# YangHai-1218/SCFlow

Measured on AMD Instinct MI355X. Metric: image-pairs/sec at 256x256, 8 GRU iters, higher is better.
Workload: dtype f32

## Files before the change

include/scflow_hip_prof.h:

```cpp
#ifndef SCFLOW_HIP_PROF_H
#define SCFLOW_HIP_PROF_H

#include "scflow_hip.h"

#ifdef __cplusplus
extern "C" {
#endif

typedef void* scf_timer_t;
int scf_timer_create(scf_timer_t* timer);
int scf_timer_destroy(scf_timer_t timer);
int scf_timer_elapsed_us(scf_timer_t timer, float* microseconds);
int scf_timer_arm(scf_timer_t timer);

int scf_conv2d_query(const scf_conv_desc* desc, int32_t* info);

enum {
  SCF_KERNEL_THIN = 1,
  SCF_KERNEL_TAPS = 2,
  SCF_KERNEL_WINO = 3,
  SCF_KERNEL_WINO1D = 4,
  SCF_KERNEL_F16X3 = 5,
  SCF_KERNEL_DMA = 6,
  SCF_KERNEL_MFMA = 7,
  SCF_KERNEL_MFMA_KSPLIT = 8,
  SCF_KERNEL_WINO_Q = 9,
  SCF_KERNEL_WINO1D4 = 10
};
typedef struct scf_conv_log_entry {
  int32_t kernel;
  int32_t Cin, Cout, KH, KW, stride, Ho, Wo, N;
  int32_t mode;
  int32_t paired;
  int32_t variant;
} scf_conv_log_entry;
int scf_conv_log_enable(int capacity);
enum {
  SCF_TUNE_WINO_VARIANT = 1,
  SCF_TUNE_DMA_FORCE_KSPLIT = 2,
  SCF_TUNE_DMA_KSPLIT_GROUPS = 3,
  SCF_TUNE_WINO1D4 = 4,
  SCF_TUNE_CONV_AUTOSLICE = 7,
  SCF_TUNE_LOOKUP_STORE = 6,
  SCF_TUNE_ITER_MERGE = 8,
  SCF_TUNE_WINO1D4_HALF = 9,
  SCF_TUNE_CONV_PAIR = 10,
  SCF_TUNE_LOOKUP_PIPE = 5
};
int scf_tune(int key, int value);
int scf_conv_log_read(scf_conv_log_entry* out, int max_entries);

#ifdef __cplusplus
}
#endif
#endif
```

scflow_amd/csrc/conv_mfma.hip:

```cpp
#include <atomic>
#include <mutex>
#include <vector>
#include "scf_common.h"

typedef float f32x16 __attribute__((ext_vector_type(16)));
typedef float f32x4 __attribute__((ext_vector_type(4)));

#include "conv_kernels.h"

template <int WM, int WN, int NCP>
__device__ __forceinline__ void mfma_taps(f32x16 (&acc)[WM][WN], const float* wl, const float* pl,
                                          const int (&boff)[WN], int T, int KW, int KC, int BM,
                                          int PW, int PHW, int half, int l32) {
  for (int t = 0; t < T; ++t) {
    const int ky = t / KW, kx = t - ky * KW;
    const float* wt = wl + (t * KC + half) * BM + l32;
    const float* pt = pl + ky * PW + kx;
#pragma unroll
    for (int c = 0; c < NCP; ++c) {
      const int cp = 2 * c;
      float a[WM], b[WN];
#pragma unroll
      for (int i = 0; i < WM; ++i) a[i] = wt[cp * BM + i * 32];
#pragma unroll
// ... 503 lines not shown

static int conv2d_walk(const scf_conv_desc* d, scf_stream_t stream, ConvReq& r) {
  ConvPlan pl;
  const int rc = conv_plan(d, &pl);
  if (rc != SCF_OK) return rc;
  const ConvK& k = pl.k;
  const int N = d->N;
  const bool dry = r.info || r.cap;
  int32_t scratch[4];
  int32_t* info = r.info ? r.info : r.cap ? scratch : nullptr;
  hipStream_t st = scf_stream(stream);
  int out = SCF_EUNSUPPORTED;
  auto took = [&](int which, int rf) { r.which = which; out = rf; return rf != SCF_EUNSUPPORTED; };
  if (d->k_slices > 1) {
    r.which = SCF_KERNEL_DMA;
    return want_dma(d) ? scf_conv_dma_dispatch(k, N, dry, info, st, r.cap) : SCF_EUNSUPPORTED;
  }
  if (took(SCF_KERNEL_THIN, scf_conv_thin_dispatch(k, N, dry, st, r.cap))) return out;
  if (d->wp_taps && took(SCF_KERNEL_TAPS, scf_conv_taps_dispatch(k, d->wp_taps, N, dry, info, st, r.cap))) return out;
  if (d->wp_wino) {
    int quarter = 0;
    const int rw = scf_conv_wino_dispatch(k, d->wp_wino, N, dry, info, st, &quarter, r.cap);
    if (took(quarter ? SCF_KERNEL_WINO_Q : SCF_KERNEL_WINO, rw)) return out;
  }
  const int w4 = g_wino1d4.load(std::memory_order_relaxed);
  if (d->wp_wino1d4 && w4 && took(SCF_KERNEL_WINO1D4, scf_conv_wino1d4_dispatch(k, d->wp_wino1d4, N, w4 == 2, dry, info, st)))
    return out;
  if (d->wp_wino1d && took(SCF_KERNEL_WINO1D, scf_conv_wino1d_dispatch(k, d->wp_wino1d, N, dry, info, st))) return out;
  if (want_f16x3(d) && took(SCF_KERNEL_F16X3, scf_conv_f16x3_dispatch(k, N, dry, info, st))) return out;
  if (want_dma(d)) {
    float* ws = nullptr;
    int64_t ws_floats = 0;
    const bool sliced = !r.info && g_autoslice.load(std::memory_order_relaxed) && kws_lookup(st, &ws, &ws_floats);
    if (sliced && !dry) {
      const int S = scf_conv_dma_autoslice(k, N);
      const int64_t per_slice = (int64_t)N * d->Cout * k.Ho * k.Wo;
      if (S > 1 && per_slice * S <= ws_floats) {
        ConvK part = k;
        part.out = ws; part.out_ns = (long long)d->Cout * k.Ho * k.Wo;
        part.bias = nullptr; part.scale = nullptr; part.shift = nullptr; part.res = nullptr; part.res_ns = 0;
        part.out_div = 1.f; part.out_div_pow2 = 1; part.act = SCF_ACT_NONE; part.act2 = SCF_ACT_NONE; part.act_split = 0;
        part.mode = SCF_CONV_PLAIN; part.gru_h = nullptr; part.gru_aux = nullptr; part.gru_z = nullptr;
        part.kslices = S; part.slice_ns = per_slice;
        r.which = SCF_KERNEL_DMA;
        const int rs = scf_conv_dma_dispatch(part, N, false, nullptr, st);
        if (rs == SCF_OK) return scf_conv_kcombine_launch(k, ws, S, per_slice, N, st);
        if (rs != SCF_EUNSUPPORTED) return rs;
      }
    }
    if (took(SCF_KERNEL_DMA, scf_conv_dma_dispatch(k, N, dry, info, st, r.cap))) {
      if (sliced && r.cap) r.cap->variant = -1;
      return out;
    }
  }
  r.which = k.ksplit ? SCF_KERNEL_MFMA_KSPLIT : SCF_KERNEL_MFMA;
  const int WM = pl.WM, WN = pl.WN;
  if (dry) {
    if (r.info) {
      r.info[0] = WM; r.info[1] = WN; r.info[2] = (int32_t)pl.nblk;
      r.info[3] = k.T * (k.KC / 2) * WM * WN / (k.ksplit ? 4 : 1);
    }
    return SCF_OK;
  }
  const int nblk = (int)pl.nblk;
  if (k.ksplit) {
    if (k.KC == 32) return launch_ksplit<32>(k, nblk, pl.lds_bytes, st);
    if (k.KC == 8) return launch_ksplit<8>(k, nblk, pl.lds_bytes, st);
    return launch_ksplit<2>(k, nblk, pl.lds_bytes, st);
  }
#define SCF_CASE(M, Nn) if (WM == M && WN == Nn) return launch_conv<M, Nn>(k, nblk, pl.lds_bytes, st);
  SCF_CASE(1, 1) SCF_CASE(1, 2) SCF_CASE(2, 1) SCF_CASE(2, 2)
  SCF_CASE(3, 1) SCF_CASE(4, 1)
#undef SCF_CASE
  return SCF_EUNSUPPORTED;
}

namespace {
std::mutex g_log_mu;
std::vector<scf_conv_log_entry> g_log;
std::atomic<int> g_log_cap{0};
}

int scf_wino_variant_set(int v);
int scf_dma_force_ksplit_set(int v);
int scf_dma_ksplit_groups_set(int v);
int scf_lookup_pipe_set(int v);
int scf_lookup_store_set(int v);
int scf_iter_merge_set(int v);
int scf_wino1d4_half_set(int v);

extern "C" int scf_tune(int key, int value) {
  if (key == SCF_TUNE_WINO_VARIANT) return scf_wino_variant_set(value);
  if (key == SCF_TUNE_DMA_FORCE_KSPLIT) return scf_dma_force_ksplit_set(value);
  if (key == SCF_TUNE_DMA_KSPLIT_GROUPS) return scf_dma_ksplit_groups_set(value);
  if (key == SCF_TUNE_LOOKUP_PIPE) return scf_lookup_pipe_set(value);
  if (key == SCF_TUNE_LOOKUP_STORE) return scf_lookup_store_set(value);
  if (key == SCF_TUNE_ITER_MERGE) return scf_iter_merge_set(value);
  if (key == SCF_TUNE_WINO1D4_HALF) return scf_wino1d4_half_set(value);
  if (key == SCF_TUNE_CONV_AUTOSLICE) {
    if (value < 0 || value > 1) return SCF_EINVAL;
    return g_autoslice.exchange(value);
  }
  if (key == SCF_TUNE_CONV_PAIR) {
    if (value < 0 || value > 1) return SCF_EINVAL;
    return g_pair_mode.exchange(value);
  }
  if (key == SCF_TUNE_WINO1D4) {
    if (value < 0 || value > 2) return SCF_EINVAL;
    return g_wino1d4.exchange(value);
  }
  return SCF_EINVAL;
}

extern "C" int scf_conv_log_enable(int capacity) {
  std::lock_guard<std::mutex> lk(g_log_mu);
  g_log.clear();
  if (capacity > 0) g_log.reserve((size_t)capacity);
  else g_log.shrink_to_fit();
  g_log_cap.store(capacity > 0 ? capacity : 0);
  return SCF_OK;
}

extern "C" int scf_conv_log_read(scf_conv_log_entry* out, int max_entries) {
  std::lock_guard<std::mutex> lk(g_log_mu);
  const int n = (int)g_log.size();
  if (out)
    for (int i = 0; i < n && i < max_entries; ++i) out[i] = g_log[(size_t)i];
  return n;
}

static void conv_log_push(const scf_conv_desc* d, int which, int paired, int variant = -1);
extern "C" int scf_conv2d(const scf_conv_desc* d, scf_stream_t stream) {
  ConvReq r;
  const int rc = conv2d_walk(d, stream, r);
  if (rc == SCF_OK) conv_log_push(d, r.which, 0);
  return rc;
}

static void conv_log_push(const scf_conv_desc* d, int which, int paired, int variant) {
  if (g_log_cap.load(std::memory_order_relaxed) <= 0) return;
  std::lock_guard<std::mutex> lk(g_log_mu);
  if ((int)g_log.size() >= g_log_cap.load()) return;
  scf_conv_log_entry e;
  e.kernel = which; e.Cin = d->C0 + d->C1; e.Cout = d->Cout; e.KH = d->KH; e.KW = d->KW; e.stride = d->stride;
  e.Ho = (d->H + 2 * d->pad_h - d->KH) / d->stride + 1;
  e.Wo = (d->W + 2 * d->pad_w - d->KW) / d->stride + 1;
  e.N = d->N; e.mode = d->mode; e.paired = paired; e.variant = variant;
  g_log.push_back(e);
}

static bool pairable(int which, const ScfLaunchCap& c) {
  switch (which) {
    case SCF_KERNEL_THIN: return true;
    case SCF_KERNEL_TAPS: return c.variant >= 1;
    case SCF_KERNEL_WINO_Q: return c.variant >= 10 && c.variant < 20;
    case SCF_KERNEL_WINO: return c.variant >= 20;
    case SCF_KERNEL_DMA: return c.variant >= 0;
    default: return false;
  }
}

static bool capture(const scf_conv_desc* d, scf_stream_t stream, ScfLaunchCap* cap, int* which) {
  ConvReq r;
  r.cap = cap;
  const bool ok = conv2d_walk(d, stream, r) == SCF_OK && pairable(r.which, *cap);
  *which = r.which;
  return ok;
}

typedef int (*PairLaunch)(const ScfLaunchCap&, const ScfLaunchCap&, hipStream_t);

static bool shared_input_form(const scf_conv_desc* a, const scf_conv_desc* b) {
  return a->in0 == b->in0 && a->C1 == 0 && b->C1 == 0 && a->C0 == b->C0 && a->N == b->N && a->H == b->H && a->W == b->W &&
         a->in0_nstride == b->in0_nstride && a->KH == 3 && a->KW == 3 && a->stride == 2 && a->pad_h == 1 && a->pad_w == 1 &&
         b->KH == 1 && b->KW == 1 && b->stride == 2 && b->pad_h == 0 && b->pad_w == 0;
// ... 158 lines not shown
```

scflow_amd/csrc/conv_wino.hip:

```cpp
#include <stdlib.h>
#include <string.h>
#include "scf_common.h"
#include "conv_kernels.h"
#include "scf_dma.h"

typedef float wn_f32x16 __attribute__((ext_vector_type(16)));
typedef float wn_f32x4 __attribute__((ext_vector_type(4)));
typedef float wn_f32x2 __attribute__((ext_vector_type(2)));

#define WN_NPI(TW, PX4) ((PX4) ? ((TW) == 2 ? 3 : 2) : ((TW) == 2 ? 8 : 5))
#define WN_KC 4
#ifndef SCF_WINO_DEFAULT_VARIANT
#define SCF_WINO_DEFAULT_VARIANT 2
#endif

#ifdef SCF_WINO_LAB
#include "wino_lab_hooks.h"
#else
#define WN_LAB(bit) 0
#define WN_LAB_FIELDS
#endif

struct WinoK {
  const float* wu;
// ... 513 lines not shown

  float* box = wn_lds + tw * (4 * 3072);
  const int cb = (f0 + (row >> 1)) * 32 + 16 * (row & 1) + 4 * half;
  float bv[8], sc[8], sh[8];
#pragma unroll
  for (int k = 0; k < 8; ++k) {
    const int co = cb + 8 * (k >> 2) + (k & 3);
    const int cc = co < p.Cout ? co : 0;
    bv[k] = p.bias ? p.bias[cc] : 0.f;
    sc[k] = p.scale ? p.scale[cc] : 1.f;
    sh[k] = p.scale ? p.shift[cc] : 0.f;
  }
  __builtin_amdgcn_sched_barrier(0);
  wn_f32x4 own[4];
#pragma unroll
  for (int qq = 0; qq < 32; qq += 2) {
    wn_f32x4 t;
#pragma unroll
    for (int h2 = 0; h2 < 2; ++h2) {
      const int f = (qq + h2) >> 4, r = (qq + h2) & 15;
      const float m0 = acc[4 * f][r], m1 = acc[4 * f + 1][r], m2 = acc[4 * f + 2][r], m3 = acc[4 * f + 3][r];
      t[2 * h2] = (m0 + m1) + m2;
      t[2 * h2 + 1] = (m1 - m2) - m3;
    }
    const int d = qq >> 3, kp = (qq & 7) >> 1;
    if (d == row) own[kp] = t;
    else *reinterpret_cast<wn_f32x4*>(box + (((row * 3 + (d < row ? d : d - 1)) * 4 + kp) * 64 + lane) * 4) = t;
  }
  __syncthreads();

  const ConvEpi e = scf_conv_epi(p, n);
  const int oy = y0 + 2 * ty, ox = x0 + 2 * tx;
  if (ox >= p.Wo || oy >= p.Ho || WN_LAB(3)) return;
  const bool row1 = oy + 1 < p.Ho;
  const bool relu = p.act == SCF_ACT_RELU;
  wn_f32x4 in[4][4];
#pragma unroll
  for (int sw = 0; sw < 4; ++sw)
#pragma unroll
    for (int kp = 0; kp < 4; ++kp) {
      if (sw == row) in[sw][kp] = own[kp];
      else in[sw][kp] = *reinterpret_cast<const wn_f32x4*>(box + (((sw * 3 + (row < sw ? row : row - 1)) * 4 + kp) * 64 + lane) * 4);
    }
  wn_f32x2 rr[8][2];
#pragma unroll
  for (int k = 0; k < 8; ++k) {
    const int co = cb + 8 * (k >> 2) + (k & 3);
    const int cc = co < p.Cout ? co : 0;
    const int off = cc * e.HWo + oy * p.Wo + ox;
#pragma unroll
    for (int i = 0; i < 2; ++i)
      rr[k][i] = (e.res && (i == 0 || row1)) ? *reinterpret_cast<const wn_f32x2*>(e.res + off + i * p.Wo) : wn_f32x2{0.f, 0.f};
  }
  __builtin_amdgcn_sched_barrier(0);
#pragma unroll
  for (int k = 0; k < 8; ++k) {
    const int co = cb + 8 * (k >> 2) + (k & 3);
    if (co >= p.Cout) continue;
    const int kp = k >> 1, h2 = 2 * (k & 1);
    wn_f32x2 y[2];
#pragma unroll
    for (int cI = 0; cI < 2; ++cI) {
      const float t0 = in[0][kp][h2 + cI], t1 = in[1][kp][h2 + cI], t3 = in[2][kp][h2 + cI], t2 = in[3][kp][h2 + cI];
      y[0][cI] = (t0 + t1) + t2;
      y[1][cI] = (t1 - t2) - t3;
    }
    const int off = co * e.HWo + oy * p.Wo + ox;
#pragma unroll
    for (int i = 0; i < 2; ++i) {
      if (i == 1 && !row1) break;
      wn_f32x2 v = {y[i][0] + bv[k], y[i][1] + bv[k]};
      if (p.scale) { v[0] = v[0] * sc[k] + sh[k]; v[1] = v[1] * sc[k] + sh[k]; }
      v[0] += rr[k][i][0]; v[1] += rr[k][i][1];
      if (relu) { v[0] = v[0] > 0.f ? v[0] : 0.f; v[1] = v[1] > 0.f ? v[1] : 0.f; }
      scf_store2<(SCF_ST_SC1 & 8) != 0>(e.out + off + i * p.Wo, v[0], v[1]);
    }
  }
}

template <int TW, bool PX4, int NR = 3, bool BURST = false>
__global__ __launch_bounds__(256 * TW, TW == 1 ? 2 : 1)
void conv_wino_q_kernel(ConvK p, WinoK q) {
  conv_wino_q_body<TW, PX4, NR, BURST>(p, q, (int)blockIdx.x, (int)gridDim.x);
}

template <bool PX4>
__global__ __launch_bounds__(256, 2)
void conv_wino_q_pair_kernel(ConvK pa, WinoK qa, ConvK pb, WinoK qb, int nba) {
  if ((int)blockIdx.x < nba) conv_wino_q_body<1, PX4>(pa, qa, (int)blockIdx.x, nba);
  else conv_wino_q_body<1, PX4>(pb, qb, (int)blockIdx.x - nba, (int)gridDim.x - nba);
}

template <bool PXA, bool PXB>
__global__ __launch_bounds__(256, 2)
void conv_wino_mixed_pair_kernel(ConvK pa, WinoK qa, ConvK pb, WinoK qb, int nba) {
  if ((int)blockIdx.x < nba) conv_wino_q_body<1, PXA>(pa, qa, (int)blockIdx.x, nba);
  else conv_wino_body<1, 2, PXB>(pb, qb, (int)blockIdx.x - nba, (int)gridDim.x - nba);
}

extern "C" int64_t scf_pack_conv_weight_wino_size(int32_t cout, int32_t cin) {
  if (cout <= 0 || cin <= 0) return 0;
  const int64_t F = (cout + 31) / 32, nchunk = (cin + WN_KC - 1) / WN_KC;
  return nchunk * 16 * F * 128;
}

extern "C" int scf_pack_conv_weight_wino(const float* w, int32_t cout, int32_t cin, float* out) {
  if (!w || !out || cout <= 0 || cin <= 0) return SCF_EINVAL;
  const int F = (cout + 31) / 32;
  memset(out, 0, sizeof(float) * (size_t)scf_pack_conv_weight_wino_size(cout, cin));
  static const double G[4][3] = {{1.0, 0.0, 0.0}, {0.5, 0.5, 0.5}, {0.5, -0.5, 0.5}, {0.0, 0.0, 1.0}};
  for (int co = 0; co < cout; ++co)
    for (int ci = 0; ci < cin; ++ci) {
      const float* g = w + ((size_t)co * cin + ci) * 9;
      double t[4][3];
      for (int i = 0; i < 4; ++i)
        for (int b = 0; b < 3; ++b) t[i][b] = G[i][0] * g[b] + G[i][1] * g[3 + b] + G[i][2] * g[6 + b];
      const int chunk = ci / WN_KC, cl = ci % WN_KC, s = cl >> 1, kh = cl & 1;
      const int frag = co / 32, m = co % 32;
      for (int i = 0; i < 4; ++i)
        for (int j = 0; j < 4; ++j) {
          const double u = t[i][0] * G[j][0] + t[i][1] * G[j][1] + t[i][2] * G[j][2];
          const int pos = 4 * (i < 2 ? i : 5 - i) + j;
          out[(((size_t)chunk * F + frag) * 16 + pos) * 128 + kh * 64 + m * 2 + s] = (float)u;
        }
    }
  return SCF_OK;
}

static std::atomic<int> g_wino_variant{0};
int scf_wino_variant_set(int v) {
#ifndef SCF_WINO_LAB
  if (v < 0 || v > 2) return SCF_EINVAL;
#else
  if (v < 0 || v > 5) return SCF_EINVAL;
#endif
  return g_wino_variant.exchange(v);
}

int scf_conv_wino_dispatch(ConvK k, const float* wu, int N, bool dry_run, int* info, hipStream_t st, int* which, ScfLaunchCap* cap) {
  if (which) *which = 0;
  if (!wu || k.KH != 3 || k.KW != 3 || k.stride != 1 || k.pad_h != 1 || k.pad_w != 1) return SCF_EUNSUPPORTED;
  if (k.w_ns != 0 || k.out_tile || k.mode != SCF_CONV_PLAIN || k.out_div != 1.0f || k.act_split > 0) return SCF_EUNSUPPORTED;
  if (k.act != SCF_ACT_NONE && k.act != SCF_ACT_RELU) return SCF_EUNSUPPORTED;
  if ((k.Wo & 1) || (k.out_ns & 1) || ((uintptr_t)k.out & 7) || (k.res && ((k.res_ns & 1) || ((uintptr_t)k.res & 7)))) return SCF_EUNSUPPORTED;
  if (k.in1 && (k.C0 % WN_KC) != 0) return SCF_EUNSUPPORTED;
  if (((uintptr_t)wu & 15) || (long long)WN_KC * k.H * k.W * 4 >= 0x7fffffffLL) return SCF_EUNSUPPORTED;
  const int F = (k.Cout + 31) / 32;
  const int tcols = (k.Wo + 1) / 2;
  int txl = 4;
  {
    int best = (tcols + 15) / 16 * 16;
    if (tcols < 16) { txl = 0; while ((1 << txl) < tcols) ++txl; if (txl < 2) txl = 2; best = 0; }
    for (int l = 3; l >= 2 && best; --l) {
      const int wpad = (tcols + (1 << l) - 1) >> l << l;
      if (wpad * 10 <= best * 9) { best = wpad; txl = l; }
    }
  }
  const int TXW = 1 << txl, TYW = 32 >> txl;
  const bool px4 = (k.W % 4) == 0 && (((uintptr_t)k.in0 | (uintptr_t)k.in1) & 15) == 0 && (k.in0_ns % 4) == 0 && (k.in1_ns % 4) == 0;
  const int cfg = px4 ? 1 : 0;
  WinoK q;
  q.wu = wu; q.F = F; q.txl = txl;
  q.nchunk = (k.Cin + WN_KC - 1) / WN_KC;
  q.sx = (k.Wo + 2 * TXW - 1) / (2 * TXW);
  auto shape = [&](int CW, int TW, int pslot) -> long long {
    q.PH = 2 * TW * TYW + 2; q.PW = px4 ? 2 * TXW + 8 : 2 * TXW + 2;
    q.PWp = q.PW + ((TXW - q.PW) & 31);
    if (WN_KC * q.PH * q.PWp > pslot) q.PWp = q.PW;
    q.PPL = q.PH * q.PWp;
    if (WN_KC * q.PPL > pslot || (F % CW) != 0) return -1;
    q.sy = (k.Ho + 2 * TW * TYW - 1) / (2 * TW * TYW);
    q.mblocks = F / CW;
    const long long nblk = (long long)N * q.sx * q.sy * q.mblocks;
    return (nblk <= 0 || nblk > 0x7fffffffLL) ? -1 : nblk;
  };
  const int min_blocks4 = scf_cu_count() / 2;
  int variant = g_wino_variant.load(std::memory_order_relaxed);
  if (variant == 0) variant = SCF_WINO_DEFAULT_VARIANT;
#ifndef SCF_WINO_LAB
  if (variant >= 3) variant = 2;
#endif
  if (variant == 2 || variant == 3 || variant == 4 || variant == 5) {
    const int TW = variant == 3 ? 2 : 1;
    const int NR = variant >= 4 ? 4 : 3;
    const bool burst = variant == 5; (void)burst;
    const int npi = WQ_NPI(TW, px4), pslot = npi * 256 * TW * (px4 ? 4 : 1);
    const long long nblk = shape(2, TW, pslot);
    if (nblk > 0 && nblk * TW >= min_blocks4) {
      if (which) *which = 1;
      size_t ldsf = (size_t)NR * (2 * 2048 + pslot);
      if (ldsf < (size_t)TW * 4 * 3072) ldsf = (size_t)TW * 4 * 3072;
      const size_t ldsb = ldsf * sizeof(float);
      if (info) { info[0] = 16; info[1] = 2 * TW; info[2] = (int)nblk; info[3] = (int)ldsb; }
      if (cap) {
        static_assert(sizeof(WinoK) <= sizeof(cap->aux), "ScfLaunchCap::aux holds a WinoK");
        cap->k = k; cap->nblk = (int)nblk; cap->ldsb = ldsb;
        memcpy(cap->aux, &q, sizeof(WinoK));
        cap->variant = (TW == 1 && NR == 3) ? 10 + cfg : -1;
        return SCF_OK;
      }
      if (dry_run) return SCF_OK;
      static std::atomic<unsigned long long> raised_q[4];
#ifdef SCF_WINO_LAB
      if (TW == 2) {
        const void* fn8 = cfg ? (const void*)conv_wino_q_kernel<2, true> : (const void*)conv_wino_q_kernel<2, false>;
        const int rc8 = scf_raise_dynamic_lds(raised_q[2 + cfg], fn8, 96 * 1024);
        if (rc8 != SCF_OK) return rc8;
        if (cfg) scf_launch((conv_wino_q_kernel<2, true>), dim3((unsigned)nblk), dim3(512), ldsb, st, k, q);
        else scf_launch((conv_wino_q_kernel<2, false>), dim3((unsigned)nblk), dim3(512), ldsb, st, k, q);
        return scf_launch_status();
      }
#endif
#ifdef SCF_WINO_LAB
      if (NR == 4 && burst) {
        static std::atomic<unsigned long long> raised_qb[2];
        const void* fnb = cfg ? (const void*)conv_wino_q_kernel<1, true, 4, true> : (const void*)conv_wino_q_kernel<1, false, 4, true>;
        const int rcb = scf_raise_dynamic_lds(raised_qb[cfg], fnb, 80 * 1024);
        if (rcb != SCF_OK) return rcb;
        if (cfg) scf_launch((conv_wino_q_kernel<1, true, 4, true>), dim3((unsigned)nblk), dim3(256), ldsb, st, k, q);
        else scf_launch((conv_wino_q_kernel<1, false, 4, true>), dim3((unsigned)nblk), dim3(256), ldsb, st, k, q);
        return scf_launch_status();
      }
      if (NR == 4) {
        static std::atomic<unsigned long long> raised_q4[2];
        const void* fn4 = cfg ? (const void*)conv_wino_q_kernel<1, true, 4> : (const void*)conv_wino_q_kernel<1, false, 4>;
        const int rc4 = scf_raise_dynamic_lds(raised_q4[cfg], fn4, 80 * 1024);
        if (rc4 != SCF_OK) return rc4;
        if (cfg) scf_launch((conv_wino_q_kernel<1, true, 4>), dim3((unsigned)nblk), dim3(256), ldsb, st, k, q);
        else scf_launch((conv_wino_q_kernel<1, false, 4>), dim3((unsigned)nblk), dim3(256), ldsb, st, k, q);
        return scf_launch_status();
      }
#endif
      const void* fn = cfg ? (const void*)conv_wino_q_kernel<1, true> : (const void*)conv_wino_q_kernel<1, false>;
      const int rc = scf_raise_dynamic_lds(raised_q[cfg], fn, 64 * 1024);
      if (rc != SCF_OK) return rc;
      if (cfg) scf_launch((conv_wino_q_kernel<1, true>), dim3((unsigned)nblk), dim3(256), ldsb, st, k, q);
      else scf_launch((conv_wino_q_kernel<1, false>), dim3((unsigned)nblk), dim3(256), ldsb, st, k, q);
      return scf_launch_status();
    }
  }
  const int CW = 1, TW = 2;
  const int npi = WN_NPI(TW, px4);
  const long long nblk = shape(CW, TW, npi * (px4 ? 1024 : 256));
  if (nblk < 0) return SCF_EUNSUPPORTED;
  if (nblk < min_blocks4) return SCF_EUNSUPPORTED;
  const size_t ldsb = (size_t)(3 * CW * 2048 + 3 * npi * (px4 ? 1024 : 256)) * sizeof(float);
  if (ldsb > 80 * 1024) return SCF_EUNSUPPORTED;
  if (info) { info[0] = 16; info[1] = CW * TW; info[2] = (int)nblk; info[3] = (int)ldsb; }
  if (cap) {
    cap->k = k; cap->nblk = (int)nblk; cap->ldsb = ldsb;
    memcpy(cap->aux, &q, sizeof(WinoK));
    cap->variant = 20 + cfg;
    return SCF_OK;
  }
  if (dry_run) return SCF_OK;
  {
    static std::atomic<unsigned long long> raised[2];
    const int rc = scf_raise_dynamic_lds(raised[cfg], cfg ? (const void*)conv_wino_kernel<1, 2, true>
                                                          : (const void*)conv_wino_kernel<1, 2, false>, 80 * 1024);
    if (rc != SCF_OK) return rc;
  }
  if (cfg) scf_launch((conv_wino_kernel<1, 2, true>), dim3((unsigned)nblk), dim3(256), ldsb, st, k, q);
  else scf_launch((conv_wino_kernel<1, 2, false>), dim3((unsigned)nblk), dim3(256), ldsb, st, k, q);
  return scf_launch_status();
}

int scf_conv_wino_pair_launch(const ScfLaunchCap& a, const ScfLaunchCap& b, hipStream_t st) {
  if (a.variant >= 10 && a.variant < 20 && b.variant >= 20 && a.nblk > 0 && b.nblk > 0) {
    const size_t ldsm = a.ldsb > b.ldsb ? a.ldsb : b.ldsb;
    WinoK qa, qb;
    memcpy(&qa, a.aux, sizeof(WinoK));
    memcpy(&qb, b.aux, sizeof(WinoK));
    const int ca = a.variant - 10, cb2 = b.variant - 20, id = ca * 2 + cb2;
    static std::atomic<unsigned long long> raised_m[4];
    const void* fn = id == 0 ? (const void*)conv_wino_mixed_pair_kernel<false, false> : id == 1 ? (const void*)conv_wino_mixed_pair_kernel<false, true>
                   : id == 2 ? (const void*)conv_wino_mixed_pair_kernel<true, false> : (const void*)conv_wino_mixed_pair_kernel<true, true>;
    const int rc = scf_raise_dynamic_lds(raised_m[id], fn, 80 * 1024);
    if (rc != SCF_OK) return rc;
    const dim3 grid((unsigned)(a.nblk + b.nblk));
    if (id == 0) scf_launch((conv_wino_mixed_pair_kernel<false, false>), grid, dim3(256), ldsm, st, a.k, qa, b.k, qb, a.nblk);
    else if (id == 1) scf_launch((conv_wino_mixed_pair_kernel<false, true>), grid, dim3(256), ldsm, st, a.k, qa, b.k, qb, a.nblk);
    else if (id == 2) scf_launch((conv_wino_mixed_pair_kernel<true, false>), grid, dim3(256), ldsm, st, a.k, qa, b.k, qb, a.nblk);
    else scf_launch((conv_wino_mixed_pair_kernel<true, true>), grid, dim3(256), ldsm, st, a.k, qa, b.k, qb, a.nblk);
    return scf_launch_status();
  }
  if (a.variant < 10 || a.variant >= 20 || a.variant != b.variant || a.nblk <= 0 || b.nblk <= 0) return SCF_EUNSUPPORTED;
  const size_t lds = a.ldsb > b.ldsb ? a.ldsb : b.ldsb;
  WinoK qa, qb;
  memcpy(&qa, a.aux, sizeof(WinoK));
  memcpy(&qb, b.aux, sizeof(WinoK));
  const int cfg = a.variant - 10;
  static std::atomic<unsigned long long> raised[2];
  const void* fn = cfg ? (const void*)conv_wino_q_pair_kernel<true> : (const void*)conv_wino_q_pair_kernel<false>;
  const int rc = scf_raise_dynamic_lds(raised[cfg], fn, 64 * 1024);
  if (rc != SCF_OK) return rc;
  const unsigned grid = (unsigned)(a.nblk + b.nblk);
  if (cfg) scf_launch((conv_wino_q_pair_kernel<true>), dim3(grid), dim3(256), lds, st, a.k, qa, b.k, qb, a.nblk);
  else scf_launch((conv_wino_q_pair_kernel<false>), dim3(grid), dim3(256), lds, st, a.k, qa, b.k, qb, a.nblk);
  return scf_launch_status();
}
```

scflow_amd/ops.py:

```python
from __future__ import annotations

import ctypes as C
import os
import math
from dataclasses import dataclass
from typing import List, Optional, Sequence, Tuple

import torch

from . import _lib
from ._lib import (ACT_NONE, ACT_RELU, ACT_SIGMOID, ACT_TANH, CONV_GRU_Q, CONV_GRU_ZR,
                   CONV_PLAIN, ConvDesc)

Tensor = torch.Tensor

__all__ = ['record_conv_kernels', 'PackedConv', 'conv_desc', 'gru_passes', 'scflow_iteration', 'side_stream_handle', 'pyramid_layout', 'untile_level', 'level_storage_shape', 'sepconv_gru', 'pack_conv_weight', 'pack_conv_weight_f16x3', 'set_conv_precision', 'set_conv_winograd', 'get_conv_winograd', 'pack_conv_weight_wino', 'pack_conv_weight_wino1d', 'pack_conv_weight_wino1d4',
           'get_conv_precision', 'set_conv_kslices', 'conv_kslices', 'conv_kslices_for', 'constant', 'clear_constants', 'register_conv_workspace', 'choose_kc', 'conv2d', 'conv2d_pair', 'corr_build', 'corr_lookup',
           'instance_norm', 'group_norm_relu', 'linear', 'fc_splitk', 'fc_slices', 'pose_update', 'reproject_flow',
           'flow_corr_2d3d', 'pnp_params', 'pnp_ransac', 'pnp',
           'unproject_depth', 'linear_pair', 'resize_bilinear', 'resize_bilinear_grad', 'reproject_flow_grad', 'pose_update_grad', 'convex_upsample', 'avgpool2x2', 'copy_channels',
           'fc_operand', 'fc_dgrad', 'fc_wgrad', 'pose_select_grad', 'group_norm_flat_grad',
           'ACT_NONE', 'ACT_RELU', 'ACT_SIGMOID', 'ACT_TANH', 'CONV_PLAIN', 'CONV_GRU_ZR',
           'CONV_GRU_Q']

# ... 579 lines not shown
            g.wp_zr_a4s, g.wp_q_a4s, g.a4s_groups = pzr.wp4s.data_ptr(), pq.wp4s.data_ptr(), pzr.g4s
        if pzr.wp4t is not None and pq.wp4t is not None and pzr.g4t == pq.g4t:
            g.wp_zr_a4t, g.wp_q_a4t, g.a4t_groups = pzr.wp4t.data_ptr(), pq.wp4t.data_ptr(), pzr.g4t
        if _CONV_WINOGRAD and not f16 and pzr.wwino1d is not None and pq.wwino1d is not None:
            g.wp_zr_wino1d, g.wp_q_wino1d = pzr.wwino1d.data_ptr(), pq.wwino1d.data_ptr()
            if pzr.wwino1d4 is not None and pq.wwino1d4 is not None:
                g.wp_zr_wino1d4, g.wp_q_wino1d4 = pzr.wwino1d4.data_ptr(), pq.wwino1d4.data_ptr()
    return arr


gru_passes = _gru_passes


def side_stream_handle() -> int:
    main = torch.cuda.current_stream()
    key = (torch.cuda.current_device(), main.cuda_stream)
    side = _SIDE.get(key)
    if side is None:
        side = _SIDE[key] = torch.cuda.Stream(device=key[0])
    return side.cuda_stream


def scflow_iteration(it: '_lib.ScflowIter') -> None:
    lib = _lib.load()
    it.lookup_timer = _LOOKUP_TIMERS.take() if _LOOKUP_TIMERS is not None else None
    _lib.check(lib.scf_scflow_iteration(C.byref(it), _stream()), 'scf_scflow_iteration')


def sepconv_gru(packs, hx: Tensor, h_channels: int, z: Tensor, rh: Tensor,
                ctx: Optional[Sequence[Tensor]] = None, ctx_channels: int = 0) -> None:
    hc = h_channels
    if ctx is not None and (ctx_channels <= 0 or len(ctx) != len(packs)):
        raise _lib.ScflowHipError('sepconv_gru: one context term per pass, ctx_channels > 0')
    if _CONV_EVENTS is not None:
        hv, xv = hx[:, :hc], hx[:, hc + ctx_channels:]
        for i, (pzr, pq) in enumerate(packs):
            if ctx is None:
                conv2d(pzr, hx, out=z, mode=CONV_GRU_ZR, gru_h=hv, gru_aux=rh)
                conv2d(pq, rh, xv, out=hv, mode=CONV_GRU_Q, gru_h=hv, gru_z=z)
            else:
                conv2d(pzr, hv, xv, out=z, mode=CONV_GRU_ZR, gru_h=hv, gru_aux=rh, res=ctx[i][:, :2 * hc])
                conv2d(pq, rh, xv, out=hv, mode=CONV_GRU_Q, gru_h=hv, gru_z=z, res=ctx[i][:, 2 * hc:])
        return
    p, n, c, h, w, sn = _nchw(hx, 'hx')
    arr = _gru_passes(packs)
    if ctx is None:
        _lib.check(_lib.load().scf_sepconv_gru(p, sn, n, hc, c - hc, h, w, arr, len(packs),
                                               _dense(z, 'z'), _dense(rh, 'rh'), _stream()),
                   'scf_sepconv_gru')
        return
    ptrs, cs = (C.c_void_p * len(ctx))(), None
    for i, t in enumerate(ctx):
        pc_, nc, cc_, hh, ww, s_ = _nchw(t, 'ctx')
        if (nc, cc_, hh, ww) != (n, 3 * hc, h, w) or (cs is not None and s_ != cs):
            raise _lib.ScflowHipError('sepconv_gru: ctx must be (N, 3*h_channels, H, W), equal strides')
        ptrs[i], cs = pc_, s_
    _lib.check(_lib.load().scf_sepconv_gru_ctx(p, sn, n, hc, ctx_channels, c - hc - ctx_channels, h, w,
                                               arr, len(packs), ptrs, cs, _dense(z, 'z'),
                                               _dense(rh, 'rh'), _stream()),
               'scf_sepconv_gru_ctx')


def _read_timers(timers):
    lib = _lib.load()
    out = []
    for tm in timers:
        us = C.c_float()
        _lib.check(lib.scf_timer_elapsed_us(tm, C.byref(us)), 'scf_timer_elapsed_us')
        lib.scf_timer_destroy(tm)
        out.append(float(us.value))
    return out


def conv_timing(enable: bool):
    global _CONV_EVENTS
    if enable:
        _CONV_EVENTS = []
        return None
    evs, _CONV_EVENTS = _CONV_EVENTS or [], None
    torch.cuda.synchronize()
    return list(zip(_read_timers([e[0] for e in evs]), [e[1] for e in evs], [e[2] for e in evs]))


TUNE_KEYS = {'wino_variant': 1, 'dma_force_ksplit': 2, 'dma_ksplit_groups': 3, 'wino1d4': 4, 'lookup_pipe': 5, 'lookup_store': 6, 'conv_autoslice': 7, 'iter_merge': 8, 'wino1d4_half': 9, 'conv_pair': 10}


def tune(key: str, value: int) -> int:
    if key not in TUNE_KEYS:
        raise ValueError(f'unknown tune key {key!r}; known: {sorted(TUNE_KEYS)}')
    prev = int(_lib.load().scf_tune(TUNE_KEYS[key], int(value)))
    if prev < 0:
        _lib.check(prev, f'scf_tune({key}, {value})')
    return prev


class record_conv_kernels:

    _active = False

    def __init__(self, capacity: int = 1 << 16) -> None:
        self.capacity, self.ran, self.paired, self.variants = capacity, [], [], []

    def __enter__(self):
        if record_conv_kernels._active:
            raise RuntimeError('record_conv_kernels does not nest (one process-wide dispatch log)')
        _lib.check(_lib.load().scf_conv_log_enable(self.capacity), 'scf_conv_log_enable')
        record_conv_kernels._active = True
        return self.ran

    def __exit__(self, *exc):
        record_conv_kernels._active = False
        lib = _lib.load()
        n = lib.scf_conv_log_read(None, 0)
        buf = (_lib.ConvLogEntry * max(n, 1))()
        n = min(lib.scf_conv_log_read(buf, n), n)
        lib.scf_conv_log_enable(0)
        for e in buf[:n]:
            self.ran.append((f'{e.Cin}->{e.Cout} {e.KH}x{e.KW}/s{e.stride} @{e.Ho}x{e.Wo} N{e.N}',
                             _lib.KERNEL_NAMES.get(e.kernel, str(e.kernel))))
            self.paired.append(e.paired)
            self.variants.append(e.variant)
        return False


def time_first_kernel(fn) -> float:
    lib = _lib.load()
    tm = C.c_void_p()
    _lib.check(lib.scf_timer_create(C.byref(tm)), 'scf_timer_create')
    lib.scf_timer_arm(tm)
    try:
        fn()
    finally:
        lib.scf_timer_arm(None)
    torch.cuda.synchronize()
    return _read_timers([tm])[0]


def pyramid_layout(h: int, w: int, radius: int = 4, num_levels: int = 4) -> int:
    return int(_lib.load().scf_corr_preferred_layout(h, w, radius, num_levels))


def level_storage_shape(h: int, w: int, level: int, tiled: bool) -> Tuple[int, int]:
    lh, lw = h >> level, w >> level
    return ((lh + 3) // 4 * 4, (lw + 7) // 8 * 8) if tiled else (lh, lw)


def untile_level(level: Tensor, lh: int, lw: int) -> Tensor:
    q, _, ph, pw = level.shape
    return (level.reshape(q, ph // 4, pw // 8, 4, 8).permute(0, 1, 3, 2, 4).reshape(q, 1, ph, pw)
            [:, :, :lh, :lw].contiguous())


def untile_level0(level0: Tensor) -> Tensor:
    return untile_level(level0, level0.shape[-2], level0.shape[-1])


def _pyramid_shapes(n: int, h: int, w: int, num_levels: int, tiled_levels: int):
    return [(n * h * w, 1, *level_storage_shape(h, w, l, bool((tiled_levels >> l) & 1)))
            for l in range(num_levels)]


def corr_build(feat1: Tensor, feat2: Tensor, num_levels: int = 4,
               out: Optional[List[Tensor]] = None, tiled_levels: int = 0) -> List[Tensor]:
    p1 = _dense(feat1, 'feat1')
    p2 = _dense(feat2, 'feat2')
    if feat1.shape != feat2.shape or feat1.dim() != 4:
        raise _lib.ScflowHipError('feat1/feat2 must be equal-shape NCHW')
# ... 1238 lines not shown
```

Before: 2352.

## Add persistent tile-looping Winograd conv kernel overlapping next-tile loads with epilogue

Adds a persistent variant of the quantized Winograd conv kernel. It launches two blocks per CU and loops over tiles. During the tail chunks of the current tile it prefetches the next tile's patch and weight data into the LDS rings, and it reuses the U ring as the exchange box, so loads overlap the epilogue and stores. Stores use buffer_store with out-of-bounds masking. It is enabled by default when there are more blocks than slots. This adds scheduling complexity and risks exposing the serial epilogue, with fewer blocks to hide latency.

```diff
diff --git a/include/scflow_hip_prof.h b/include/scflow_hip_prof.h
--- a/include/scflow_hip_prof.h
+++ b/include/scflow_hip_prof.h
@@ -45,6 +45,7 @@
   SCF_TUNE_ITER_MERGE = 8,
   SCF_TUNE_WINO1D4_HALF = 9,
   SCF_TUNE_CONV_PAIR = 10,
+  SCF_TUNE_WINO_TILE_LOOP = 11,
   SCF_TUNE_LOOKUP_PIPE = 5
 };
 int scf_tune(int key, int value);
diff --git a/scflow_amd/csrc/conv_mfma.hip b/scflow_amd/csrc/conv_mfma.hip
--- a/scflow_amd/csrc/conv_mfma.hip
+++ b/scflow_amd/csrc/conv_mfma.hip
@@ -609,6 +609,7 @@
 }
 
 int scf_wino_variant_set(int v);
+int scf_wino_tile_loop_set(int v);
 int scf_dma_force_ksplit_set(int v);
 int scf_dma_ksplit_groups_set(int v);
 int scf_lookup_pipe_set(int v);
@@ -618,6 +619,7 @@
 
 extern "C" int scf_tune(int key, int value) {
   if (key == SCF_TUNE_WINO_VARIANT) return scf_wino_variant_set(value);
+  if (key == SCF_TUNE_WINO_TILE_LOOP) return scf_wino_tile_loop_set(value);
   if (key == SCF_TUNE_DMA_FORCE_KSPLIT) return scf_dma_force_ksplit_set(value);
   if (key == SCF_TUNE_DMA_KSPLIT_GROUPS) return scf_dma_ksplit_groups_set(value);
   if (key == SCF_TUNE_LOOKUP_PIPE) return scf_lookup_pipe_set(value);
diff --git a/scflow_amd/csrc/conv_wino.hip b/scflow_amd/csrc/conv_wino.hip
--- a/scflow_amd/csrc/conv_wino.hip
+++ b/scflow_amd/csrc/conv_wino.hip
@@ -619,6 +619,361 @@
 __global__ __launch_bounds__(256 * TW, TW == 1 ? 2 : 1)
 void conv_wino_q_kernel(ConvK p, WinoK q) {
   conv_wino_q_body<TW, PX4, NR, BURST>(p, q, (int)blockIdx.x, (int)gridDim.x);
+}
+
+#define WQL_NST 16
+
+__device__ __forceinline__ void scf_bstore_b64(scf_rsrc4 rsrc, unsigned voff, wn_f32x2 v) {
+  asm volatile("buffer_store_dwordx2 %0, %1, %2, 0 offen" : : "v"(v), "v"(voff), "s"(rsrc) : "memory");
+}
+
+template <bool PX4>
+__global__ __launch_bounds__(256, 2)
+void conv_wino_q_loop_kernel(ConvK p, WinoK q, int nblk) {
+  extern __shared__ __attribute__((aligned(16))) float wn_lds[];
+  constexpr int NT = 256, NR = 3;
+  constexpr int USLOT = 2 * 2048;
+  constexpr int NUI = 4;
+  constexpr int NPI = WQ_NPI(1, PX4);
+  constexpr int PSLOT = NPI * NT * (PX4 ? 4 : 1);
+  constexpr int GRP = NUI + NPI;
+  static_assert(NR * USLOT == 4 * 3072, "the exchange box is exactly the U ring: the patch ring stays free for the next tile");
+  const int tid = threadIdx.x, lane = tid & 63;
+  const int row = __builtin_amdgcn_readfirstlane(tid >> 6);
+  const int half = lane >> 5, l32 = lane & 31;
+  const int grid = (int)gridDim.x;
+  const int TXW = 1 << q.txl, TYW = 32 >> q.txl;
+  const int HW = p.H * p.W;
+
+  float* Us = wn_lds;
+  float* Ps = Us + NR * USLOT;
+  const unsigned u_lds = scf_lds_addr(Us), p_lds = scf_lds_addr(Ps);
+
+  auto locate = [&](int logical, int& mb_, int& n_, int& y0_, int& x0_) {
+    int lb = scf_xcd_remap(logical, nblk);
+    mb_ = __builtin_amdgcn_readfirstlane(lb % q.mblocks);
+    lb /= q.mblocks;
+    const int xs = __builtin_amdgcn_readfirstlane(lb % q.sx);
+    lb /= q.sx;
+    const int ys = __builtin_amdgcn_readfirstlane(lb % q.sy);
+    n_ = __builtin_amdgcn_readfirstlane(lb / q.sy);
+    y0_ = ys * (2 * TYW);
+    x0_ = xs * (2 * TXW);
+  };
+
+  unsigned pvo[NPI];
+  auto set_pvo = [&](int y0_, int x0_) {
+    const int NC = PX4 ? q.PWp >> 2 : q.PWp, PPC = q.PH * NC;
+    const float rPPC = 1.0f / (float)PPC, rNC = 1.0f / (float)NC;
+#pragma unroll
+    for (int i = 0; i < NPI; ++i) {
+      const int e = i * NT + tid;
+      const int c = wn_div(e, PPC, rPPC), r = e - c * PPC;
+      const int py = wn_div(r, NC, rNC), px = r - py * NC;
+      const int iy = y0_ - 1 + py, ix = PX4 ? x0_ - 4 + 4 * px : x0_ - 1 + px;
+      const bool ok = c < WN_KC && iy >= 0 && iy < p.H && ix >= 0 && ix < p.W && (PX4 || px < q.PW);
+      pvo[i] = ok ? (unsigned)((c * HW + iy * p.W + ix) * 4) : SCF_BUF_OOB;
+    }
+  };
+  unsigned uvo[NUI], uld[NUI];
+#pragma unroll
+  for (int i = 0; i < NUI; ++i) {
+    const int j = row + 4 * i;
+    const int f = j >> 3, part = j & 7;
+    uvo[i] = (unsigned)(f * 8192 + part * 1024 + lane * 16);
+    uld[i] = (unsigned)(f * 8192 + part * 1024);
+  }
+  const unsigned u_chunk_bytes = (unsigned)(q.F * 8192);
+  const unsigned u_total = (unsigned)q.nchunk * u_chunk_bytes;
+  scf_rsrc4 urs;
+  int u_left;
+  auto arm_u = [&](int mb_) {
+    const unsigned skip = (unsigned)mb_ * 16384u;
+    urs = scf_make_rsrc(reinterpret_cast<const char*>(q.wu) + skip, u_total - skip);
+    u_left = (int)(u_total - skip);
+  };
+  auto issue_u = [&](int slot) {
+    const unsigned dst = u_lds + (unsigned)(slot * USLOT * 4);
+#pragma unroll
+    for (int i = 0; i < NUI; ++i) scf_bdma_b128(urs, uvo[i], dst + uld[i]);
+    const unsigned lo = (unsigned)urs[0] + u_chunk_bytes;
+    urs[1] += lo < u_chunk_bytes ? 1 : 0;
+    urs[0] = (int)lo;
+    u_left -= (int)u_chunk_bytes;
+    urs[2] = u_left > 0 ? u_left : 0;
+  };
+  const unsigned p_chunk_bytes = (unsigned)(WN_KC * HW * 4);
+  const float* p_seg;
+  int p_left;
+  bool p_second;
+  scf_rsrc4 prs;
+  auto arm_p = [&](int n_) {
+    p_seg = p.in0 + (long long)n_ * p.in0_ns;
+    p_left = p.C0;
+    p_second = p.in1 == nullptr;
+    prs = scf_make_rsrc(p_seg, (unsigned)((p_left < WN_KC ? p_left : WN_KC) * HW * 4));
+  };
+  int n = 0;
+  auto issue_p = [&](int slot) {
+    const unsigned dst = p_lds + (unsigned)((slot * PSLOT + row * (PX4 ? 256 : 64)) * 4);
+#pragma unroll
+    for (int i = 0; i < NPI; ++i) {
+      if (PX4) scf_bdma_b128(prs, pvo[i], dst + (unsigned)(i * NT * 16));
+      else scf_bdma_b32(prs, pvo[i], dst + (unsigned)(i * NT * 4));
+    }
+    p_left -= WN_KC;
+    if (p_left <= 0 && !p_second) {
+      p_second = true;
+      p_seg = p.in1 + (long long)n * p.in1_ns;
+      p_left = p.Cin - p.C0;
+      prs = scf_make_rsrc(p_seg, 0u);
+    } else {
+      const unsigned lo = (unsigned)prs[0] + p_chunk_bytes;
+      prs[1] += lo < p_chunk_bytes ? 1 : 0;
+      prs[0] = (int)lo;
+    }
+    const int cl = p_left < WN_KC ? p_left : WN_KC;
+    prs[2] = cl > 0 ? cl * HW * 4 : 0;
+  };
+
+  const int ty = l32 >> q.txl, tx = l32 & (TXW - 1);
+  const int ra = row == 0 ? 0 : row == 3 ? 2 : 1, rb = row == 2 ? 3 : row == 3 ? 1 : 2;
+  const float sigma = row == 1 ? 1.0f : -1.0f;
+  const wn_f32x2 sigma2 = {sigma, sigma};
+  unsigned prow[2][2];
+  {
+    const int poff = half * q.PPL + 2 * ty * q.PWp + 2 * tx + (PX4 ? 3 : 0);
+#pragma unroll
+    for (int sI = 0; sI < 2; ++sI) {
+      prow[sI][0] = p_lds + (unsigned)((poff + 2 * sI * q.PPL + ra * q.PWp) * 4);
+      prow[sI][1] = p_lds + (unsigned)((poff + 2 * sI * q.PPL + rb * q.PWp) * 4);
+    }
+  }
+  wn_f32x2 dws[2][2][2];
+  auto win_load = [&](unsigned slot_bytes, int sI) {
+#pragma unroll
+    for (int i = 0; i < 2; ++i) {
+      const __attribute__((address_space(3))) float* r =
+          (const __attribute__((address_space(3))) float*)(uintptr_t)(prow[sI][i] + slot_bytes);
+      dws[sI][i][0] = wn_f32x2{r[0], r[1]};
+      dws[sI][i][1] = wn_f32x2{r[2], r[3]};
+    }
+  };
+  auto win_transform = [&](wn_f32x2 (&bo)[2][2], int sI) {
+    wn_f32x2 v01, v23;
+    asm("v_pk_fma_f32 %0, %1, %2, %3" : "=v"(v01) : "v"(sigma2), "v"(dws[sI][1][0]), "v"(dws[sI][0][0]));
+    asm("v_pk_fma_f32 %0, %1, %2, %3" : "=v"(v23) : "v"(sigma2), "v"(dws[sI][1][1]), "v"(dws[sI][0][1]));
+    asm("v_pk_add_f32 %0, %1, %2 op_sel:[0,0] op_sel_hi:[1,0] neg_lo:[0,1]" : "=v"(bo[sI][0]) : "v"(v01), "v"(v23));
+    asm("v_pk_add_f32 %0, %1, %2 op_sel:[0,1] op_sel_hi:[1,1] neg_lo:[0,1] neg_hi:[1,0]" : "=v"(bo[sI][1]) : "v"(v23), "v"(v01));
+  };
+  const float* ua = Us + row * 512 + lane * 2;
+  float* box = wn_lds;
+
+  int t = (int)blockIdx.x;
+  int mb, y0, x0;
+  locate(t, mb, n, y0, x0);
+  set_pvo(y0, x0);
+  arm_u(mb);
+  arm_p(n);
+  int s0 = 0;
+  bool first = true;
+  issue_p(0); issue_u(0);
+  issue_u(1); issue_p(1);
+  issue_u(2); issue_p(2);
+  scf_wait_vmcnt_imm<GRP>();
+
+  for (;;) {
+    const int tn = t + grid;
+    const bool more = tn < nblk;
+    int mbn = 0, nn = 0, y0n = 0, x0n = 0, s0n = 0;
+    const int n_cur = n;
+
+    wn_f32x16 acc[8];
+    __syncthreads();
+    wn_f32x2 a0[8], a1[8], b0[2][2], b1[2][2];
+    {
+      const float* u0 = ua + s0 * USLOT;
+#pragma unroll
+      for (int x = 0; x < 8; ++x) a0[x] = *reinterpret_cast<const wn_f32x2*>(u0 + (x >> 2) * 2048 + (x & 3) * 128);
+      win_load((unsigned)(s0 * PSLOT * 4), 0); win_transform(b0, 0);
+      win_load((unsigned)(s0 * PSLOT * 4), 1); win_transform(b0, 1);
+    }
+    __syncthreads();
+
+    int s1 = s0 == NR - 1 ? 0 : s0 + 1;
+    auto chunk = [&](auto kind_tag, const wn_f32x2 (&a)[8], const wn_f32x2 (&b)[2][2], wn_f32x2 (&an)[8], wn_f32x2 (&bn)[2][2], const int c) {
+      constexpr int KIND = decltype(kind_tag)::value;
+      constexpr bool GEN = KIND != 0;
+      const wn_f32x16 zero16 = {0.f, 0.f, 0.f, 0.f, 0.f, 0.f, 0.f, 0.f, 0.f, 0.f, 0.f, 0.f, 0.f, 0.f, 0.f, 0.f};
+      const float* uc = ua + s1 * USLOT;
+      const unsigned pcb = (unsigned)(s1 * PSLOT * 4);
+#define WQ_M(X, S)                                                                                             \
+      acc[X] = __builtin_amdgcn_mfma_f32_32x32x2f32(a[X][S], b[S][((X) & 3) >> 1][(X) & 1],                      \
+                                                    (KIND == 2 && (S) == 0) ? zero16 : acc[X], 0, 0, 0);         \
+      __builtin_amdgcn_sched_barrier(0);
+      int s3 = s1 + NR - 1;
+      s3 = s3 >= NR ? s3 - NR : s3;
+      const bool tail = GEN && more && c + NR >= q.nchunk;
+      WQ_M(0, 0)
+      win_load(pcb, 0);
+      __builtin_amdgcn_sched_barrier(0);
+      WQ_M(1, 0)
+      win_load(pcb, 1);
+      __builtin_amdgcn_sched_barrier(0);
+      WQ_M(2, 0)
+      if (!tail) issue_u(s3);
+      __builtin_amdgcn_sched_barrier(0);
+      WQ_M(3, 0)
+      if (tail && c + NR == q.nchunk) {
+        locate(tn, mbn, nn, y0n, x0n);
+        n = nn;
+        arm_p(nn);
+        set_pvo(y0n, x0n);
+        s0n = s3;
+        asm volatile("s_nop 4");
+      }
+      issue_p(s3);
+      __builtin_amdgcn_sched_barrier(0);
+      WQ_M(4, 0)
+#pragma unroll
+      for (int x = 0; x < 8; ++x) an[x] = *reinterpret_cast<const wn_f32x2*>(uc + (x >> 2) * 2048 + (x & 3) * 128);
+      __builtin_amdgcn_sched_barrier(0);
+      WQ_M(5, 0)
+      win_transform(bn, 0);
+      __builtin_amdgcn_sched_barrier(0);
+      WQ_M(6, 0) WQ_M(7, 0)
+      WQ_M(0, 1) WQ_M(1, 1)
+      win_transform(bn, 1);
+      __builtin_amdgcn_sched_barrier(0);
+      WQ_M(2, 1) WQ_M(3, 1) WQ_M(4, 1) WQ_M(5, 1) WQ_M(6, 1) WQ_M(7, 1)
+#undef WQ_M
+      const bool st = KIND == 2 && !first;
+      if (tail) {
+        if (st) scf_wait_vmcnt_imm<NPI + WQL_NST>();
+        else scf_wait_vmcnt_imm<NPI>();
+      } else {
+        if (st) scf_wait_vmcnt_imm<GRP + WQL_NST>();
+        else scf_wait_vmcnt_imm<GRP>();
+      }
+      __syncthreads();
+      s1 = s1 == NR - 1 ? 0 : s1 + 1;
+    };
+    constexpr std::integral_constant<int, 0> steady;
+    constexpr std::integral_constant<int, 1> gen;
+    chunk(std::integral_constant<int, 2>(), a0, b0, a1, b1, 0);
+    int c = 1;
+    const int tail0 = q.nchunk - NR > 1 ? q.nchunk - NR : 1;
+    for (; c + 1 < tail0; c += 2) {
+      chunk(steady, a1, b1, a0, b0, c);
+      chunk(steady, a0, b0, a1, b1, c + 1);
+    }
+    if (c < tail0) {
+      chunk(steady, a1, b1, a0, b0, c);
+      ++c;
+#pragma unroll
+      for (int x = 0; x < 8; ++x) a1[x] = a0[x];
+#pragma unroll
+      for (int x = 0; x < 2; ++x) { b1[x][0] = b0[x][0]; b1[x][1] = b0[x][1]; }
+    }
+    if (c < q.nchunk) { chunk(gen, a1, b1, a0, b0, c); ++c; }
+    if (c < q.nchunk) { chunk(gen, a0, b0, a1, b1, c); ++c; }
+    if (c < q.nchunk) { chunk(gen, a1, b1, a0, b0, c); ++c; }
+    if (!more) scf_wait_vmcnt_imm<0>();
+    __syncthreads();
+
+    const ConvEpi e = scf_conv_epi(p, n_cur);
+    const scf_rsrc4 ors = scf_make_rsrc(e.out, (unsigned)(p.Cout * e.HWo * 4));
+    const int cb = (mb * 2 + (row >> 1)) * 32 + 16 * (row & 1) + 4 * half;
+    float bv[8], sc[8], sh[8];
+#pragma unroll
+    for (int k = 0; k < 8; ++k) {
+      const int co = cb + 8 * (k >> 2) + (k & 3);
+      const int cc = co < p.Cout ? co : 0;
+      bv[k] = p.bias ? p.bias[cc] : 0.f;
+      sc[k] = p.scale ? p.scale[cc] : 1.f;
+      sh[k] = p.scale ? p.shift[cc] : 0.f;
+    }
+    __builtin_amdgcn_sched_barrier(0);
+    wn_f32x4 own[4];
+#pragma unroll
+    for (int qq = 0; qq < 32; qq += 2) {
+      wn_f32x4 tt;
+#pragma unroll
+      for (int h2 = 0; h2 < 2; ++h2) {
+        const int f = (qq + h2) >> 4, r = (qq + h2) & 15;
+        const float m0 = acc[4 * f][r], m1 = acc[4 * f + 1][r], m2 = acc[4 * f + 2][r], m3 = acc[4 * f + 3][r];
+        tt[2 * h2] = (m0 + m1) + m2;
+        tt[2 * h2 + 1] = (m1 - m2) - m3;
+      }
+      const int d = qq >> 3, kp = (qq & 7) >> 1;
+      if (d == row) own[kp] = tt;
+      else *reinterpret_cast<wn_f32x4*>(box + (((row * 3 + (d < row ? d : d - 1)) * 4 + kp) * 64 + lane) * 4) = tt;
+    }
+    __syncthreads();
+    wn_f32x4 in[4][4];
+#pragma unroll
+    for (int sw = 0; sw < 4; ++sw)
+#pragma unroll
+      for (int kp = 0; kp < 4; ++kp) {
+        if (sw == row) in[sw][kp] = own[kp];
+        else in[sw][kp] = *reinterpret_cast<const wn_f32x4*>(box + (((sw * 3 + (row < sw ? row : row - 1)) * 4 + kp) * 64 + lane) * 4);
+      }
+    if (more) {
+      __syncthreads();
+      arm_u(mbn);
+      asm volatile("s_nop 4");
+      int s = s0n;
+      issue_u(s);
+      s = s == NR - 1 ? 0 : s + 1;
+      issue_u(s);
+      s = s == NR - 1 ? 0 : s + 1;
+      issue_u(s);
+    }
+    __builtin_amdgcn_sched_barrier(0);
+
+    const int oy = y0 + 2 * ty, ox = x0 + 2 * tx;
+    const bool valid = ox < p.Wo && oy < p.Ho;
+    const bool row1 = oy + 1 < p.Ho;
+    const bool relu = p.act == SCF_ACT_RELU;
+    const int pix = valid ? oy * p.Wo + ox : 0;
+    const int pix1 = pix + (valid && row1 ? p.Wo : 0);
+    wn_f32x2 rr[8][2];
+#pragma unroll
+    for (int k = 0; k < 8; ++k) {
+      const int co = cb + 8 * (k >> 2) + (k & 3);
+      const int cc = co < p.Cout ? co : 0;
+      rr[k][0] = e.res ? *reinterpret_cast<const wn_f32x2*>(e.res + cc * e.HWo + pix) : wn_f32x2{0.f, 0.f};
+      rr[k][1] = e.res ? *reinterpret_cast<const wn_f32x2*>(e.res + cc * e.HWo + pix1) : wn_f32x2{0.f, 0.f};
+    }
+    __builtin_amdgcn_sched_barrier(0);
+    asm volatile("s_nop 4");
+#pragma unroll
+    for (int k = 0; k < 8; ++k) {
+      const int co = cb + 8 * (k >> 2) + (k & 3);
+      const bool cok = valid && co < p.Cout;
+      const int kp = k >> 1, h2 = 2 * (k & 1);
+      wn_f32x2 y[2];
+#pragma unroll
+      for (int cI = 0; cI < 2; ++cI) {
+        const float t0 = in[0][kp][h2 + cI], t1 = in[1][kp][h2 + cI], t3 = in[2][kp][h2 + cI], t2 = in[3][kp][h2 + cI];
+        y[0][cI] = (t0 + t1) + t2;
+        y[1][cI] = (t1 - t2) - t3;
+      }
+      const int off = co * e.HWo + oy * p.Wo + ox;
+#pragma unroll
+      for (int i = 0; i < 2; ++i) {
+        wn_f32x2 v = {y[i][0] + bv[k], y[i][1] + bv[k]};
+        if (p.scale) { v[0] = v[0] * sc[k] + sh[k]; v[1] = v[1] * sc[k] + sh[k]; }
+        v[0] += rr[k][i][0]; v[1] += rr[k][i][1];
+        if (relu) { v[0] = v[0] > 0.f ? v[0] : 0.f; v[1] = v[1] > 0.f ? v[1] : 0.f; }
+        scf_bstore_b64(ors, (cok && (i == 0 || row1)) ? (unsigned)((off + i * p.Wo) * 4) : SCF_BUF_OOB, v);
+      }
+    }
+    if (!more) break;
+    t = tn; mb = mbn; y0 = y0n; x0 = x0n; s0 = s0n;
+    first = false;
+    scf_wait_vmcnt_imm<NUI + WQL_NST>();
+  }
 }
 
 template <bool PX4>
@@ -672,6 +1027,15 @@
   if (v < 0 || v > 5) return SCF_EINVAL;
 #endif
   return g_wino_variant.exchange(v);
+}
+
+#ifndef SCF_WINO_TILE_LOOP_DEFAULT
+#define SCF_WINO_TILE_LOOP_DEFAULT 1
+#endif
+static std::atomic<int> g_wino_tile_loop{SCF_WINO_TILE_LOOP_DEFAULT};
+int scf_wino_tile_loop_set(int v) {
+  if (v < 0 || v > 1) return SCF_EINVAL;
+  return g_wino_tile_loop.exchange(v);
 }
 
 int scf_conv_wino_dispatch(ConvK k, const float* wu, int N, bool dry_run, int* info, hipStream_t st, int* which, ScfLaunchCap* cap) {
@@ -768,6 +1132,17 @@
         return scf_launch_status();
       }
 #endif
+      const int slots = 2 * scf_cu_count();
+      if (g_wino_tile_loop.load(std::memory_order_relaxed) && nblk > slots && q.nchunk >= 3 &&
+          (long long)k.Cout * k.Ho * k.Wo * 4 < 0x7fffffffLL) {
+        static std::atomic<unsigned long long> raised_l[2];
+        const void* fnl = cfg ? (const void*)conv_wino_q_loop_kernel<true> : (const void*)conv_wino_q_loop_kernel<false>;
+        const int rcl = scf_raise_dynamic_lds(raised_l[cfg], fnl, 64 * 1024);
+        if (rcl != SCF_OK) return rcl;
+        if (cfg) scf_launch((conv_wino_q_loop_kernel<true>), dim3((unsigned)slots), dim3(256), ldsb, st, k, q, (int)nblk);
+        else scf_launch((conv_wino_q_loop_kernel<false>), dim3((unsigned)slots), dim3(256), ldsb, st, k, q, (int)nblk);
+        return scf_launch_status();
+      }
       const void* fn = cfg ? (const void*)conv_wino_q_kernel<1, true> : (const void*)conv_wino_q_kernel<1, false>;
       const int rc = scf_raise_dynamic_lds(raised_q[cfg], fn, 64 * 1024);
       if (rc != SCF_OK) return rc;
diff --git a/scflow_amd/ops.py b/scflow_amd/ops.py
--- a/scflow_amd/ops.py
+++ b/scflow_amd/ops.py
@@ -685,7 +685,7 @@
     return list(zip(_read_timers([e[0] for e in evs]), [e[1] for e in evs], [e[2] for e in evs]))
 
 
-TUNE_KEYS = {'wino_variant': 1, 'dma_force_ksplit': 2, 'dma_ksplit_groups': 3, 'wino1d4': 4, 'lookup_pipe': 5, 'lookup_store': 6, 'conv_autoslice': 7, 'iter_merge': 8, 'wino1d4_half': 9, 'conv_pair': 10}
+TUNE_KEYS = {'wino_variant': 1, 'dma_force_ksplit': 2, 'dma_ksplit_groups': 3, 'wino1d4': 4, 'lookup_pipe': 5, 'lookup_store': 6, 'conv_autoslice': 7, 'iter_merge': 8, 'wino1d4_half': 9, 'conv_pair': 10, 'wino_tile_loop': 11}
 
 
 def tune(key: str, value: int) -> int:
```

Measured after the change: 2374 (median of 6 runs). No clear change (+0.9%).
